# gopro/cineform-sdk

Measured on AMD Instinct MI355X. Metric: 1080p YUY2 encode+decode fps, higher is better.
Workload: dtype int16

## Files before the change

cineform-sdk_amd/csrc/cfhd_batch.cpp:

```cpp
#include "../../include/cfhd_amd.h"
#include "cfhd_core.h"
#include "cfhd_bitstream.h"
#include "cfhd_device.h"
#include "cfhd_metadata.h"
#include "cfhd_params.h"
#include <string.h>
#include <stdlib.h>
#include <vector>
#include <thread>
#include <atomic>
#include <chrono>
#include <memory>

using namespace cfhd;

struct cfhd_amd_chunk { EncodeBatch enc; DecodeBatch dec; int first = 0, n = 0; };

struct cfhd_amd_batch {
	FramePlan plan;
	int n = 0, nthreads = 1, quality = 4, pixel_kind = PIX_YUY2;
	int color_format = 2, color_space = 2; bool progressive = true;
	bool decode = true;
	std::vector<std::unique_ptr<cfhd_amd_chunk>> chunks;
	cfhd_amd_chunk &chunk_of(int i, int *local) { for (auto &c : chunks) if (i < c->first + c->n) { *local = i - c->first; return *c; } *local = 0; return *chunks[0]; }
// ... 36 lines not shown
	static const int forced = [] { const char *e = getenv("CFHD_AMD_QUEUE"); return e && strcmp(e, "ordered") == 0 ? 2 : (e && strcmp(e, "free") == 0 ? 0 : -1); }();
	const int turns = forced >= 0 ? forced : (b->decode ? 0 : 1);
	const bool ordered = turns >= 1, ordered_decode = turns >= 2;
	if (ordered && stage_order_wait(c->enc.device(), 0, c->enc.stream())) return -2;
	if (b->host_in && c->enc.upload_frames(b->host_in, b->host_in_stride, b->host_in_pitch)) return -2;
	if (c->enc.launch_forward(false)) return -2;
	for (int l = 0; l < c->n; l++) {
		SampleHeaderInfo h = { base_number + (uint32_t)(c->first + l) + 1, b->color_format, b->color_space, b->quality, b->progressive, b->frame_meta[c->first + l].data(), b->frame_meta[c->first + l].size(), nullptr, 0 };
		if (c->enc.entropy().set_frame_header(l, h)) return -6;
	}
	if (c->enc.entropy().launch()) return -2;
	if (ordered && stage_order_done(c->enc.device(), 0, c->enc.stream())) return -2;
	if (b->decode) {
		if (ordered_decode && stage_order_wait(c->enc.device(), 1, c->dec.stream())) return -5;
		c->dec.entropy().set_producer_events(c->enc.entropy().headers_event(), c->enc.entropy().samples_event());
		if (c->dec.entropy().set_samples_device(c->enc.entropy().device_sample(0), c->enc.entropy().sample_cap(), c->enc.entropy().device_sizes())) return -4;
		if (c->dec.launch_entropy() || c->dec.launch_inverse(seed + (uint32_t)c->first)) return -5;
		if (ordered_decode && stage_order_done(c->enc.device(), 1, c->dec.stream())) return -5;
		if (b->host_out && c->dec.download_frames(b->host_out, b->host_out_stride, b->host_out_pitch)) return -5;
	}
	if (c->enc.entropy().download_queue()) return -2;
	b->t_launched = now();
	return 0;
}
long long batch_finish(cfhd_amd_batch *b)
{
	cfhd_amd_chunk *c = b->chunks[0].get();
	if (c->enc.entropy().download_finish() || c->enc.wait()) return -2;
	bool overflow = false, peaks = false;
	for (int l = 0; l < c->n; l++) {
		size_t n = c->enc.entropy().sample_bytes(l); b->sample_size[c->first + l] = n;
// ... 112 lines not shown
		const int rc = batch_launch(b);
		if (rc) return rc;
		return batch_finish(b);
	} else if (b->gpu_entropy && b->device_handoff) {
		prepare_meta();
		std::atomic<int> err(0);
		std::vector<double> t_sub(b->chunks.size(), 0.0), t_enc(b->chunks.size(), 0.0);
		parallel_for((int)b->chunks.size(), (int)b->chunks.size(), [&](int k) {
			cfhd_amd_chunk *c = b->chunks[k].get();
			auto fail = [&](int code) { int z = 0; err.compare_exchange_strong(z, code); };
			if (c->enc.launch_forward(false)) return fail(-2);
			for (int l = 0; l < c->n; l++) if (c->enc.entropy().set_frame_header(l, header(c->first + l))) return fail(-6);
			if (c->enc.entropy().launch()) return fail(-2);
			if (b->decode) {
				c->dec.entropy().set_producer_events(c->enc.entropy().headers_event(), c->enc.entropy().samples_event());
				if (c->dec.entropy().set_samples_device(c->enc.entropy().device_sample(0), c->enc.entropy().sample_cap(), c->enc.entropy().device_sizes())) return fail(-4);
				if (c->dec.launch_entropy() || c->dec.launch_inverse(seed + (uint32_t)c->first)) return fail(-5);
			}
			t_sub[k] = now();
			if (c->enc.entropy().download() || c->enc.wait()) return fail(-2);
			for (int l = 0; l < c->n; l++) {
				size_t n = c->enc.entropy().sample_bytes(l); b->sample_size[c->first + l] = n; if (!n) { fail(-3); continue; }
				if (c->enc.entropy().needs_peak_table(l)) fail(-8);
			}
			t_enc[k] = now();
			if (b->decode) { if (c->dec.wait()) return fail(-5); if (c->dec.entropy().check()) return fail(-7); }
		});
		if (err.load()) return err.load();
		t1 = t0; t2 = t0;
		for (size_t k = 0; k < b->chunks.size(); k++) { if (t_sub[k] > t1) t1 = t_sub[k]; if (t_enc[k] > t2) t2 = t_enc[k]; }
		if (t2 < t1) t2 = t1;
// ... 188 lines not shown
```

cineform-sdk_amd/csrc/cfhd_entropy_gpu.h:

```cpp
#pragma once
#include "cfhd_core.h"
#include "cfhd_bitstream.h"
#include "cfhd_gop.h"
#include <vector>

namespace cfhd {

int device_stream_create(void **stream);
void device_stream_destroy(void *stream);
void device_stream_release(void *stream);
void device_streams_lean(bool on);
bool device_streams_are_lean();
struct StreamScope { StreamScope(); explicit StreamScope(void *preset ); ~StreamScope(); void *stream() const; };


class GpuEntropyEncoder {
public:
	GpuEntropyEncoder();
	~GpuEntropyEncoder();
	int prepare(const FramePlan &plan, int nframes, int16_t *d_coeffs, size_t coeff_stride_elems, size_t sample_cap, void *stream);
	int set_frame_header(int i, const SampleHeaderInfo &hdr);
	void set_plan(const FramePlan &plan) { plan_ = plan; }
	int prepare_group(const GopPlan &plan, int ngroups, int16_t *d_coeffs, size_t coeff_stride_elems, size_t sample_cap, void *stream);
	void set_group_plan(const GopPlan &plan) { gplan_ = plan; }
	int launch();
	int download();
	int download_queue();
	int download_finish();
	int fetch_sizes();
	const uint32_t *device_sizes() const { return d_sizes_; }
	const uint8_t *host_sample(int i) const { return h_samples_ + h_offsets_[i]; }
	uint8_t *device_sample(int i) { return d_samples_ + (size_t)i * cap_; }
	uint32_t sample_bytes(int i) const { return h_sizes_[i]; }
	void set_active(int k) { active_ = k; }
	void set_speculative_download(bool on) { speculative_download_ = on; if (!on) expect_bytes_ = 0; }
	bool needs_peak_table(int i) const { return peak_flags_in_use() && (h_sizes_[n_ + i] & 2u) != 0; }
	bool has_peak_table(int i) const { return peak_flags_in_use() && (h_sizes_[n_ + i] & 1u) != 0; }
	bool peak_flags_in_use() const { return group_ ? gplan_.interlaced : plan_.interlaced; }
	size_t sample_cap() const { return cap_; }
	int total_segments() const { return total_segs_; }
	float kernel_ms(int k);
	void set_level1_event(void *ev) { ev_level1_ = ev; }
	void *block_slots() const { return d_blocks_; }
	unsigned long long *block_masks(int frame) const { return d_masks_ ? d_masks_ + (size_t)frame * masks_per_frame_ : nullptr; }
	void set_block_lists(bool on) { use_blocks_ = on && d_blocks_; }
	bool block_lists() const { return use_blocks_; }
	void *headers_event() const { return ev_[3]; }
	void *samples_event() const { return ev_[4]; }
private:
	struct Host; Host *host_;
	void release();
	int prepare_units(int n, int16_t *d_coeffs, size_t coeff_stride_elems, size_t sample_cap, void *stream);
	void build_template(const SampleHeaderInfo &hdr, SampleTemplate *t) const;
	bool group_ = false; GopPlan gplan_;
	FramePlan plan_; int n_ = 0, active_ = 0, device_ = 0 ; size_t cap_ = 0; void *stream_ = nullptr;
	int active_frames() const { return active_ > 0 && active_ < n_ ? active_ : n_; }
	int nbands_ = 0, total_segs_ = 0; size_t tok_per_frame_ = 0;
	std::vector<SampleTemplate> tmpl_;
	uint8_t *d_samples_ = nullptr, *h_samples_ = nullptr;
	uint32_t *d_sizes_ = nullptr, *h_sizes_ = nullptr;
	uint8_t *d_packed_ = nullptr; uint32_t *d_offsets_ = nullptr, *h_offsets_ = nullptr;
	size_t expect_bytes_ = 0, copied_ahead_ = 0; int expect_frames_ = 0; bool speculative_download_ = false;
	void *d_tables_ = nullptr, *d_bands_ = nullptr, *d_segband_ = nullptr, *d_segs_ = nullptr, *d_bandstate_ = nullptr, *d_frames_ = nullptr, *d_tokens_ = nullptr;
	uint8_t *d_tmpl_ = nullptr, *h_tmpl_ = nullptr;
	bool dirty_ = true;
	void *ev_[5] = {nullptr, nullptr, nullptr, nullptr, nullptr}; bool timed_ = false;
	bool split_ = false, serial_split_ = false; void *ev_level1_ = nullptr, *stream2_ = nullptr, *ev2_[3] = {nullptr, nullptr, nullptr};
	int16_t *d_coeffs_ = nullptr; size_t coeff_stride_ = 0;
	void *d_blocks_ = nullptr; unsigned long long *d_masks_ = nullptr; size_t masks_per_frame_ = 0; bool use_blocks_ = false;
};


class GpuEntropyDecoder {
public:
	GpuEntropyDecoder();
	~GpuEntropyDecoder();
	void set_interlaced(bool on) { interlaced_ = on; }
	void set_active(int k) { active_ = k; }
	void set_skip_level1(bool skip) { skip_level1_ = skip; }
	int prepare(const FramePlan &plan, int nframes, int16_t *d_coeffs, size_t coeff_stride_elems, size_t sample_cap, int out_pixel_kind, void *stream);
	int set_sample_host(int i, const uint8_t *sample, size_t size);
	int set_sample_device(int i, const uint8_t *d_sample, const uint8_t *host_copy, size_t size);
	int set_samples_device(const uint8_t *d_samples, size_t stride_bytes, const uint32_t *d_sizes);
	void set_producer_events(void *headers, void *payloads) { ev_headers_ = headers; ev_payloads_ = payloads; }
	int launch();
	int check();
	float kernel_ms(int k);
	bool chunk_indexed() const { return dx_; }
	void *levels23_event() const { return l23_split_ ? ev_l23_ : nullptr; }
	void set_block_lists(bool on) { use_blocks_ = on && d_masks_; }
	bool level1_as_block_lists() const { return blocks_written_; }
	void dense_pyramid_uploaded() { blocks_written_ = false; }
	const unsigned long long *block_masks(int frame) const { return d_masks_ ? d_masks_ + (size_t)frame * masks_per_frame_ : nullptr; }
	int stats(uint32_t out[16]);
private:
	struct Host; Host *host_;
	void release();
	FramePlan plan_; int n_ = 0, out_kind_ = 0; size_t cap_ = 0, coeff_stride_ = 0; void *stream_ = nullptr;
	int16_t *d_coeffs_ = nullptr;
	uint8_t *d_samples_ = nullptr, *h_samples_ = nullptr;
	void *d_tables_ = nullptr, *d_bandjobs_ = nullptr, *d_lowjobs_ = nullptr, *d_plan_ = nullptr;
	void *ev_headers_ = nullptr, *ev_payloads_ = nullptr;
	bool skip_level1_ = false, interlaced_ = false; void *d_diffjobs_ = nullptr;
	int active_ = 0;
	int active_frames() const { return active_ > 0 && active_ < n_ ? active_ : n_; }
	const uint8_t *ext_samples_ = nullptr; size_t ext_stride_ = 0; const uint32_t *ext_sizes_ = nullptr;
	int *d_errors_ = nullptr, *h_errors_ = nullptr;
	bool lane_kernel_ = false;
	bool dx_ = true;
	void *d_tile_start_ = nullptr, *d_stats_ = nullptr, *d_repair_ = nullptr, *d_alts_ = nullptr, *d_reindex_ = nullptr, *d_alt_entries_ = nullptr; uint32_t alt_slots_ = 0;
	void *d_idx_tables_ = nullptr, *d_entries_ = nullptr, *d_recs_ = nullptr, *d_chunk_base_ = nullptr, *d_chunk_job_ = nullptr, *d_sums_ = nullptr, *d_counters_ = nullptr;
	uint32_t max_chunks_ = 0, *h_counters_ = nullptr; void *h_chunk_job_ = nullptr;
	int grid_index_ = 0, grid_tiles_ = 0;
	int device_ = 0;
	int launch_dx(bool device_jobs, int njobs, uint32_t host_chunks, int lowpass_jobs);
	void *ev_l23_ = nullptr, *ev_low_ = nullptr; bool l23_split_ = false;
	void *ev_[8] = {nullptr, nullptr, nullptr, nullptr, nullptr, nullptr, nullptr, nullptr}; bool timed_ = false;
	bool parse_end_ = false;
	unsigned long long *d_masks_ = nullptr; size_t masks_per_frame_ = 0; bool use_blocks_ = false, blocks_written_ = false;
};

// ... 19 lines not shown
```

cineform-sdk_amd/csrc/cfhd_entropy_gpu.hip:

```cpp
#include "cfhd_entropy_gpu.h"
#include "cfhd_entropy_jobs.h"
#include <hip/hip_runtime.h>
#include <string.h>
#include <stdio.h>
#include <stdlib.h>
#include <algorithm>

namespace cfhd {

int device_init();
int device_current();
namespace { int g_fail(hipError_t e, const char *what) { fprintf(stderr, "[cfhd_amd] %s: %s\n", what, hipGetErrorString(e)); return (int)e ? (int)e : -1; } }
#define HIPCHK(expr) do { hipError_t _e = (expr); if (_e != hipSuccess) return g_fail(_e, #expr); } while (0)

struct GpuEntropyEncoder::Host { EntHostJobs jobs; std::vector<EntHoleGeom> geom; dev::EntFrameJob *frames = nullptr;  };

GpuEntropyEncoder::GpuEntropyEncoder() : host_(new Host) {}
GpuEntropyEncoder::~GpuEntropyEncoder() { release(); delete host_; }

void GpuEntropyEncoder::release()
{
	(void)hipSetDevice(device_);
	void *dev[] = { d_samples_, d_sizes_, d_tables_, d_bands_, d_segband_, d_segs_, d_bandstate_, d_frames_, d_tmpl_, d_packed_, d_offsets_, d_tokens_, d_blocks_, d_masks_ };
	for (void *p : dev) if (p) (void)hipFree(p);
	if (h_samples_) (void)hipHostFree(h_samples_);
	if (h_sizes_) (void)hipHostFree(h_sizes_);
	if (h_offsets_) (void)hipHostFree(h_offsets_);
	d_packed_ = nullptr; d_offsets_ = h_offsets_ = nullptr;
	if (h_tmpl_) (void)hipHostFree(h_tmpl_);
	if (host_->frames) { (void)hipHostFree(host_->frames); host_->frames = nullptr; }
	for (void *&e : ev_) if (e) { (void)hipEventDestroy((hipEvent_t)e); e = nullptr; }
	for (void *&e : ev2_) if (e) { (void)hipEventDestroy((hipEvent_t)e); e = nullptr; }
	if (stream2_) { device_stream_destroy(stream2_); stream2_ = nullptr; }
	timed_ = false;
	d_samples_ = h_samples_ = nullptr; d_sizes_ = h_sizes_ = nullptr; d_tables_ = d_bands_ = d_segband_ = d_segs_ = d_bandstate_ = d_frames_ = d_tokens_ = nullptr;
	d_tmpl_ = h_tmpl_ = nullptr; n_ = 0;
	d_blocks_ = nullptr; d_masks_ = nullptr; masks_per_frame_ = 0; use_blocks_ = false;
}

int GpuEntropyEncoder::prepare(const FramePlan &plan, int nframes, int16_t *d_coeffs, size_t stride, size_t sample_cap, void *stream)
{
	group_ = false; plan_ = plan;
	return prepare_units(nframes, d_coeffs, stride, sample_cap, stream);
}

int GpuEntropyEncoder::prepare_group(const GopPlan &plan, int ngroups, int16_t *d_coeffs, size_t stride, size_t sample_cap, void *stream)
{
	group_ = true; gplan_ = plan; plan_ = FramePlan(); plan_.interlaced = false;
	return prepare_units(ngroups, d_coeffs, stride, sample_cap, stream);
}
// ... 31 lines not shown
	HIPCHK(hipMalloc(&d_bands_, jobs.bands.size() * sizeof(dev::EntBandJob)));
	HIPCHK(hipMemcpy(d_bands_, jobs.bands.data(), jobs.bands.size() * sizeof(dev::EntBandJob), hipMemcpyHostToDevice));
	HIPCHK(hipMalloc(&d_segband_, jobs.segjobs.size() * sizeof(dev::EntSegJob)));
	HIPCHK(hipMemcpy(d_segband_, jobs.segjobs.data(), jobs.segjobs.size() * sizeof(dev::EntSegJob), hipMemcpyHostToDevice));
	HIPCHK(hipMalloc(&d_segs_, jobs.segjobs.size() * sizeof(dev::EntSegState)));
	HIPCHK(hipMalloc(&d_tokens_, jobs.tok_per_frame * (size_t)n_ * sizeof(uint32_t)));
	HIPCHK(hipMalloc(&d_bandstate_, jobs.bands.size() * sizeof(dev::EntBandState)));
	static_assert((int)kBlockChunkCols == (int)dev::FWD_CHUNK_COLS_ENT, "one chunk geometry");
	if (lists) {
		int mask_base[kMaxChannels][kNumBands];
		masks_per_frame_ = (size_t)block_list_layout(plan, mask_base);
		HIPCHK(hipMalloc(&d_blocks_, stride * 2 * (size_t)n_));
		HIPCHK(hipMalloc((void **)&d_masks_, masks_per_frame_ * 8 * (size_t)n_ + 64));
		HIPCHK(hipMemset(d_masks_, 0, masks_per_frame_ * 8 * (size_t)n_ + 64));
	}
	HIPCHK(hipMalloc((void **)&d_samples_, cap_ * n_));
	HIPCHK(hipHostMalloc((void **)&h_samples_, cap_ * n_, hipHostMallocPortable));
	HIPCHK(hipMalloc((void **)&d_sizes_, sizeof(uint32_t) * 2 * n_));
	HIPCHK(hipHostMalloc((void **)&h_sizes_, sizeof(uint32_t) * 2 * n_, hipHostMallocPortable));
	memset(h_sizes_, 0, sizeof(uint32_t) * 2 * n_);
	HIPCHK(hipMalloc((void **)&d_packed_, cap_ * n_));
	HIPCHK(hipMalloc((void **)&d_offsets_, sizeof(uint32_t) * (n_ + 1)));
	HIPCHK(hipHostMalloc((void **)&h_offsets_, sizeof(uint32_t) * (n_ + 1), hipHostMallocPortable));
	memset(h_offsets_, 0, sizeof(uint32_t) * (n_ + 1));
	HIPCHK(hipMalloc((void **)&d_tmpl_, (size_t)kEntTmplStride * n_));
	HIPCHK(hipHostMalloc((void **)&h_tmpl_, (size_t)kEntTmplStride * n_, hipHostMallocPortable));
	memset(h_tmpl_, 0, (size_t)kEntTmplStride * n_);
	HIPCHK(hipMalloc(&d_frames_, n_ * sizeof(dev::EntFrameJob)));
	HIPCHK(hipHostMalloc((void **)&host_->frames, n_ * sizeof(dev::EntFrameJob), hipHostMallocPortable));
	for (int f = 0; f < n_; f++) { SampleHeaderInfo h = hdr0; h.frame_number = (uint32_t)f + 1; if ((rc = set_frame_header(f, h))) return rc; }
	for (void *&e : ev_) HIPCHK(hipEventCreate((hipEvent_t *)&e));
	for (void *&e : ev2_) HIPCHK(hipEventCreate((hipEvent_t *)&e));
	if (n_ >= 8 || !device_streams_are_lean()) HIPCHK((hipError_t)device_stream_create(&stream2_));
	return 0;
}

int GpuEntropyEncoder::set_frame_header(int f, const SampleHeaderInfo &hdr)
{
	if (f < 0 || f >= n_) return -1;
	SampleTemplate &t = tmpl_[f];
	build_template(hdr, &t);
	if (!ent_fill_frame_block(host_->geom, t, f, host_->jobs, d_coeffs_ + (size_t)f * coeff_stride_, h_tmpl_ + (size_t)kEntTmplStride * f)) return -4;
	host_->frames[f] = ent_frame_job(t, d_tmpl_ + (size_t)kEntTmplStride * f, d_samples_ + cap_ * f, (uint32_t)cap_, d_sizes_ + f, d_sizes_ + n_ + f);
	dirty_ = true;
	return 0;
}

int GpuEntropyEncoder::launch()
{
	(void)hipSetDevice(device_);
	hipStream_t st = (hipStream_t)stream_;
	if (dirty_) {
		HIPCHK(hipMemcpyAsync(d_tmpl_, h_tmpl_, (size_t)kEntTmplStride * n_, hipMemcpyHostToDevice, st));
		HIPCHK(hipMemcpyAsync(d_frames_, host_->frames, n_ * sizeof(dev::EntFrameJob), hipMemcpyHostToDevice, st));
		dirty_ = false;
	}
	const dev::EntTables *T = (const dev::EntTables *)d_tables_;
	const dev::EntBatchGeom geom = { total_segs_ / n_, nbands_, coeff_stride_, tok_per_frame_ };
// ... 31 lines not shown
		HIPCHK(hipStreamWaitEvent(s2, (hipEvent_t)ev_level1_, 0));
		if (peak_flags_in_use()) HIPCHK(hipMemsetAsync(d_sizes_ + n_, 0, sizeof(uint32_t) * n_, s2));
		HIPCHK(hipEventRecord((hipEvent_t)ev2_[0], s2));
		for (const auto &r : host_->jobs.ranges_l1) count_range(s2, r.first, r.second, true);
		HIPCHK(hipEventRecord((hipEvent_t)ev2_[1], s2));
		for (const auto &r : host_->jobs.ranges_rest) count_range(st, r.first, r.second);
		HIPCHK(hipEventRecord((hipEvent_t)ev2_[2], st));
		HIPCHK(hipStreamWaitEvent(st, (hipEvent_t)ev2_[1], 0));
	} else if (use_blocks_) {
		for (const auto &r : host_->jobs.ranges_l1) count_range(st, r.first, r.second, true);
		for (const auto &r : host_->jobs.ranges_rest) count_range(st, r.first, r.second);
	} else count_range(st, 0, total_segs_ / n_);
	HIPCHK(hipEventRecord((hipEvent_t)ev_[1], st));
	dev::k_ent_scan<<<nbands_ * act, dev::ENT_THREADS, 0, st>>>((const dev::EntBandJob *)d_bands_, (dev::EntSegState *)d_segs_, (dev::EntBandState *)d_bandstate_, T);
	HIPCHK(hipEventRecord((hipEvent_t)ev_[2], st));
	const unsigned layout_parts = act >= 256 ? 8u : (unsigned)((2048 + act - 1) / act > 256 ? 256 : (2048 + act - 1) / act);
	dev::k_ent_layout<<<dim3((unsigned)act, layout_parts), dev::ENT_THREADS, 0, st>>>((const dev::EntFrameJob *)d_frames_, (const dev::EntBandJob *)d_bands_, (dev::EntSegState *)d_segs_,
	                                                  (dev::EntBandState *)d_bandstate_, T);
	HIPCHK(hipEventRecord((hipEvent_t)ev_[3], st));
	{
		dev::EntPeakHoles which; which.n = 0;
		for (size_t h = 0; h < tmpl_[0].holes.size() && which.n < 7; h++) if (tmpl_[0].holes[h].kind == 2) which.hole[which.n++] = (int)h;
		if (which.n) dev::k_ent_peaks<<<dim3(act >= 64 ? 4u : 32u, (unsigned)which.n, (unsigned)act), dev::ENT_THREADS, 0, st>>>((const dev::EntFrameJob *)d_frames_, which, (const dev::EntBandJob *)d_bands_,
		                                                  (const dev::EntSegJob *)d_segband_, geom, (const dev::EntSegState *)d_segs_, (const dev::EntBandState *)d_bandstate_);
	}
#ifdef CFHD_AMD_PROBES
	const int emit_probe = []{ const char *e = getenv("CFHD_AMD_EMIT_PROBE"); return e ? atoi(e) : 0; }();
#else
	const int emit_probe = 0;
#endif
// ... 23 lines not shown
{
	(void)hipSetDevice(device_);
	hipStream_t st = (hipStream_t)stream_;
	HIPCHK(hipMemcpyAsync(h_sizes_, d_sizes_, sizeof(uint32_t) * 2 * n_, hipMemcpyDeviceToHost, st));
	HIPCHK(hipStreamSynchronize(st));
	return 0;
}

int GpuEntropyEncoder::download() { const int rc = download_queue(); return rc ? rc : download_finish(); }

int GpuEntropyEncoder::download_queue()
{
	(void)hipSetDevice(device_);
	hipStream_t st = (hipStream_t)stream_;
	const bool direct = false;
	(void)hipGetLastError();
	const int act = active_frames();
	dev::k_ent_pack_offsets<<<1, dev::ENT_THREADS, 0, st>>>(d_sizes_, act, d_offsets_);
	dev::k_ent_pack<<<dim3(direct ? 2 : 8, (unsigned)act), dev::ENT_THREADS, 0, st>>>(d_samples_, cap_, d_sizes_, d_offsets_, direct ? h_samples_ : d_packed_);
	HIPCHK(hipGetLastError());
	HIPCHK(hipMemcpyAsync(h_sizes_, d_sizes_, sizeof(uint32_t) * 2 * n_, hipMemcpyDeviceToHost, st));
	HIPCHK(hipMemcpyAsync(h_offsets_, d_offsets_, sizeof(uint32_t) * (act + 1), hipMemcpyDeviceToHost, st));
	copied_ahead_ = 0;
	if (!direct && expect_bytes_ && expect_frames_ == act) {
		copied_ahead_ = expect_bytes_ < cap_ * (size_t)act ? expect_bytes_ : cap_ * (size_t)act;
		HIPCHK(hipMemcpyAsync(h_samples_, d_packed_, copied_ahead_, hipMemcpyDeviceToHost, st));
	}
	return 0;
}

int GpuEntropyEncoder::download_finish()
{
	(void)hipSetDevice(device_);
	hipStream_t st = (hipStream_t)stream_;
	const bool direct = false;
// ... 103 lines not shown
		HIPCHK(hipMalloc(&d_plan_, sizeof(dp)));
		HIPCHK(hipMemcpy(d_plan_, &dp, sizeof(dp), hipMemcpyHostToDevice));
	}
	if (dx_ && plan.encoded_format == ENC_YUV422 && plan.num_channels == 3) {
		int mask_base[kMaxChannels][kNumBands];
		masks_per_frame_ = (size_t)dec_block_list_layout(plan, mask_base);
		HIPCHK(hipMalloc((void **)&d_masks_, masks_per_frame_ * 8 * (size_t)n_));
	}
	host_->bands.assign(n_, {}); host_->lows.assign(n_, {}); host_->diffs.assign(n_, {}); host_->host_bytes.assign(n_, 0);
	for (void *&e : ev_) HIPCHK(hipEventCreate((hipEvent_t *)&e));
	HIPCHK(hipEventCreate((hipEvent_t *)&ev_l23_));
	HIPCHK(hipEventCreate((hipEvent_t *)&ev_low_));
	return 0;
}

int GpuEntropyDecoder::set_samples_device(const uint8_t *d_samples, size_t stride_bytes, const uint32_t *d_sizes)
{
	if (!d_samples || !d_sizes || (stride_bytes & 255) || ((uintptr_t)d_samples & 255)) return -1;
	ext_samples_ = d_samples; ext_stride_ = stride_bytes; ext_sizes_ = d_sizes;
	return 0;
}

int GpuEntropyDecoder::set_sample_host(int i, const uint8_t *sample, size_t size)
{
	if (i < 0 || i >= n_ || size > cap_) return -1;
	memcpy(h_samples_ + cap_ * i, sample, size);
	int rc = set_sample_device(i, d_samples_ + cap_ * i, sample, size);
	if (rc == 0) host_->host_bytes[i] = (size + 3) & ~(size_t)3;
	return rc;
}

int GpuEntropyDecoder::set_sample_device(int i, const uint8_t *d_sample, const uint8_t *host_copy, size_t size)
{
	if (i < 0 || i >= n_) return -1;
// ... 21 lines not shown
int GpuEntropyDecoder::launch()
{
	(void)hipSetDevice(device_);
	hipStream_t st = (hipStream_t)stream_;
	l23_split_ = false; blocks_written_ = false;
	if (ext_samples_) {
		const int nch = plan_.num_channels, nb = n_ * nch * 9;
		HIPCHK(hipMemsetAsync(d_errors_, 0, sizeof(int), st));
		(void)hipGetLastError();
		static const bool parse_early = [] { const char *e = getenv("CFHD_AMD_PARSE_EARLY"); return !(e && atoi(e) == 0); }();
		if (!parse_early && ev_payloads_) ev_headers_ = ev_payloads_;
		if (ev_headers_) HIPCHK(hipStreamWaitEvent(st, (hipEvent_t)ev_headers_, 0));
		HIPCHK(hipEventRecord((hipEvent_t)ev_[0], st));
		dev::k_dec_parse<<<n_, dev::DEC_PARSE_THREADS, 0, st>>>(ext_samples_, ext_stride_, ext_sizes_, n_,
			(const dev::DecPlan *)d_plan_, d_coeffs_, coeff_stride_, (dev::DecBandJob *)d_bandjobs_, (dev::DecLowpassJob *)d_lowjobs_, d_errors_,
			interlaced_ && dx_ ? (dev::DecDiffJob *)d_diffjobs_ : nullptr);
		parse_end_ = ev_payloads_ != nullptr;
		if (parse_end_) { HIPCHK(hipEventRecord((hipEvent_t)ev_[4], st)); HIPCHK(hipStreamWaitEvent(st, (hipEvent_t)ev_payloads_, 0)); }
		ev_headers_ = ev_payloads_ = nullptr;
		HIPCHK(hipEventRecord((hipEvent_t)ev_[1], st));
		l23_split_ = false;
		if (dx_) { const int rc_dx = launch_dx(true, nb, 0u, n_ * nch); if (rc_dx) return rc_dx; }
		else if (n_ <= kLowLatencyFrames) dev::k_dec_bands_par_ll<<<nb, dev::DECP_LL_THREADS, 0, st>>>((const dev::DecBandJob *)d_bandjobs_, (const dev::DecTables *)d_tables_, d_errors_);
		else dev::k_dec_bands_par<<<nb, dev::DECP_THREADS, 0, st>>>((const dev::DecBandJob *)d_bandjobs_, (const dev::DecTables *)d_tables_, d_errors_);
		HIPCHK(hipEventRecord((hipEvent_t)ev_[2], st));
		if (!l23_split_) dev::k_dec_lowpass<<<dim3(8, (unsigned)(n_ * nch)), 256, 0, st>>>((const dev::DecLowpassJob *)d_lowjobs_);
		HIPCHK(hipGetLastError());
		HIPCHK(hipEventRecord((hipEvent_t)ev_[3], st));
		timed_ = true;
		HIPCHK(hipMemcpyAsync(h_errors_, d_errors_, sizeof(int), hipMemcpyDeviceToHost, st));
		return 0;
// ... 269 lines not shown
```

cineform-sdk_amd/csrc/cfhd_entropy_jobs.h:

```cpp
#pragma once
#include "cfhd_core.h"
#include "cfhd_bitstream.h"
#include "cfhd_gop.h"
#include "cfhd_entropy_kernels.h"
#include "cfhd_dec_kernels.h"
#include <vector>
#include <algorithm>
#include <string.h>

namespace cfhd {

enum { kEntTmplBytes = 6144, kEntWordHolesBytes = 1536, kEntHolesBytes = dev::ENT_MAX_HOLES * (int)sizeof(dev::EntHole), kEntMaxPatches = 96,
       kEntPatchBytes = kEntMaxPatches * (int)sizeof(dev::EntPatch), kEntTmplStride = kEntTmplBytes + kEntWordHolesBytes + kEntHolesBytes + kEntPatchBytes };

inline void ent_build_tables(dev::EntTables *h, int codebook = 1)
{
	const EntropyTables *t = entropy_tables(codebook);
	memcpy(h->value_code, t->value_code, sizeof(h->value_code));
	memcpy(h->run_bits, t->run_bits, sizeof(h->run_bits));
	for (int c = 0; c < 3072; c++) { h->run_count[c] = t->run_count[c]; h->run_size[c] = t->run_size[c]; }
	h->run_total[0] = 0;
	for (int c = 1; c < 3072; c++) h->run_total[c] = (uint16_t)(t->run_size[c] + h->run_total[c - t->run_count[c]]);
	h->band_end_bits = t->band_end_bits; h->band_end_size = t->band_end_size;
	for (int c = 0; c < 3072; c++) { h->run_pack[c].x = t->run_bits[c]; h->run_pack[c].y = (uint32_t)t->run_size[c] | ((uint32_t)t->run_count[c] << 8); }
// ... 271 lines not shown
		d.lp_width = bd.width; d.lp_height = bd.height; d.lp_pitch = bd.pitch;
	}
	dev::EntPatch *ep = (dev::EntPatch *)(block + kEntTmplBytes + kEntWordHolesBytes + kEntHolesBytes);
	for (size_t i = 0; i < t.patches.size(); i++) {
		const SampleTemplate::Patch &p = t.patches[i];
		ep[i].kind = p.kind; ep[i].at_tmpl = p.at_tmpl; ep[i].at_holes = p.at_holes; ep[i].start_tmpl = p.start_tmpl; ep[i].start_holes = p.start_holes;
		ep[i].end_tmpl = p.end_tmpl; ep[i].end_holes = p.end_holes; ep[i].tag = p.tag;
	}
	return true;
}
inline bool ent_fill_frame_block(const FramePlan &plan, const SampleTemplate &t, int f, const EntHostJobs &jobs, const int16_t *coeffs_f, uint8_t *block)
{
	return ent_fill_frame_block(ent_hole_geometry(plan, t), t, f, jobs, coeffs_f, block);
}

inline dev::EntFrameJob ent_frame_job(const SampleTemplate &t, uint8_t *block_addr, uint8_t *out, uint32_t out_cap, uint32_t *size_out, uint32_t *peak_flag)
{
	dev::EntFrameJob fj;
	fj.out = out; fj.out_cap = out_cap;
	fj.tmpl = block_addr; fj.tmpl_bytes = (int)t.bytes.size();
	fj.word_holes = block_addr + kEntTmplBytes;
	fj.holes = (const dev::EntHole *)(block_addr + kEntTmplBytes + kEntWordHolesBytes); fj.nholes = (int)t.holes.size();
	fj.patches = (const dev::EntPatch *)(block_addr + kEntTmplBytes + kEntWordHolesBytes + kEntHolesBytes); fj.npatches = (int)t.patches.size();
	fj.sample_bytes = size_out; fj.peak_flag = peak_flag;
	return fj;
}


inline bool dec_build_jobs(const ParsedSample &ps, const FramePlan &plan, const uint8_t *sample_addr, int16_t *coeff_base, int out_pixel_kind,
                           std::vector<dev::DecBandJob> *bands, std::vector<dev::DecLowpassJob> *lowpass, bool skip_level1 = false)
{
	for (int c = 0; c < plan.num_channels; c++) {
		const ParsedBand &lp = ps.lowpass[c];
		const BandDesc &ll = plan.ch[c].band[2][0];
// ... 113 lines not shown
```

cineform-sdk_amd/csrc/cfhd_entropy_kernels.h:

```cpp
#pragma once
#include <stdint.h>
#include <cfhd_gfx950.h>

#ifdef CFHD_AMD_PROBES
#define CFHD_PROBE(p) (p)
#else
#define CFHD_PROBE(p) 0
#endif

namespace cfhd {
namespace dev {

#ifndef CFHD_ENT_FILL
#define CFHD_ENT_FILL 16384
#endif
#ifndef CFHD_ENT_PER_THREAD
#define CFHD_ENT_PER_THREAD 16
#endif
#ifndef CFHD_ENT_TOK_CAP
#define CFHD_ENT_TOK_CAP 256
#endif
enum { FWD_CHUNK_COLS_ENT = 496 };
enum { ENT_THREADS = 256, ENT_LANES = 64, ENT_WAVES = ENT_THREADS / ENT_LANES, ENT_PER_THREAD = CFHD_ENT_PER_THREAD, ENT_SEG = ENT_LANES * ENT_PER_THREAD,
       ENT_LDS_WORDS = 1024, ENT_TOK_CAP = CFHD_ENT_TOK_CAP, ENT_MAX_HOLES = 60 ,
// ... 53 lines not shown

struct EntBandState { uint32_t seg_bits, tail_run, payload_bytes, base_byte; uint8_t *out;
                      uint32_t npeaks, pad; uint8_t *peak_out;  };

struct EntHole { int tmpl_offset, kind, fixed_bytes, band_job; const int16_t *lowpass; int lp_width, lp_height, lp_pitch; };
struct EntPatch { int kind, at_tmpl, at_holes, start_tmpl, start_holes, end_tmpl, end_holes, tag; };

struct EntFrameJob {
	uint8_t *out; uint32_t out_cap;
	const uint8_t *tmpl; int tmpl_bytes;
	const uint8_t *word_holes;
	const EntHole *holes; int nholes;
	const EntPatch *patches; int npatches;
	uint32_t *sample_bytes;
	uint32_t *peak_flag;
};

__device__ __forceinline__ uint32_t bswap32(uint32_t v) { return (v >> 24) | ((v >> 8) & 0xff00u) | ((v << 8) & 0xff0000u) | (v << 24); }

__device__ __forceinline__ int block_excl_sum(int v, int *buf, int *total)
{
	const int lane = wave_lane(), wave = (int)(threadIdx.x >> 6);
	const int incl = (int)wave_incl_scan((uint32_t)v);
	if (lane == ENT_LANES - 1) buf[wave] = incl;
	__syncthreads();
	int base = 0, tot = 0;
#pragma unroll
	for (int w = 0; w < ENT_WAVES; w++) { const int x = buf[w]; if (w < wave) base += x; tot += x; }
	if (total) *total = tot;
	__syncthreads();
// ... 359 lines not shown
		b.base_byte = 0; b.out = nullptr;
		b.npeaks = carry_peaks; b.pad = 0; b.peak_out = nullptr;
	}
}

__device__ __forceinline__ void put_code_plain(uint32_t *words, uint64_t pos, uint32_t code, int size)
{
	if (!size) return;
	const uint64_t v = (uint64_t)code << (64 - size - (int)(pos & 31));
	uint32_t *w = words + (pos >> 5);
	w[0] |= bswap32((uint32_t)(v >> 32));
	const uint32_t lo = (uint32_t)v;
	if (lo) w[1] |= bswap32(lo);
}

__global__ void __launch_bounds__(ENT_THREADS) k_ent_layout(const EntFrameJob *frames, const EntBandJob *bands, EntSegState *segs,
                                                             EntBandState *band_state, const EntTables *tables)
{
	const EntFrameJob &f = frames[blockIdx.x];
	const int part = blockIdx.y, nparts = gridDim.y;
	__shared__ uint32_t s_cum[ENT_MAX_HOLES + 1];
	__shared__ uint32_t s_piece[ENT_MAX_HOLES + 1];
	__shared__ int s_ok;
	const int tid = threadIdx.x;
	if (tid < 64) {
		uint32_t bytes = 0;
		if (tid < f.nholes) {
			const EntHole &hole = f.holes[tid];
			if (hole.kind == 0) bytes = (uint32_t)hole.fixed_bytes;
			else if (hole.kind == 1) bytes = band_state[hole.band_job].payload_bytes;
			else {
				const uint32_t np = band_state[hole.band_job].npeaks;
				bytes = (np && np <= (uint32_t)ENT_PEAK_TABLE_MAX) ? 4u + 4u * ((np + 1u) >> 1) : 0u;
			}
		}
		const uint32_t pieces = tid < f.nholes ? (bytes / ENT_FILL ? bytes / ENT_FILL : 1u) : 0u;
		const uint32_t cum = wave_incl_scan(bytes), pc = wave_incl_scan(pieces);
		if (tid <= f.nholes && tid <= ENT_MAX_HOLES) { s_cum[tid] = cum - bytes; s_piece[tid] = pc - pieces; }
		const uint32_t total = (uint32_t)f.tmpl_bytes + wave_get(cum, 63);
		if (tid == 0) { s_ok = total <= f.out_cap; if (part == 0) *f.sample_bytes = total <= f.out_cap ? total : 0u; }
	}
	__syncthreads();
	if (!s_ok) return;
	uint32_t *out = (uint32_t *)f.out;
	const uint32_t *tw = (const uint32_t *)f.tmpl;
	if (part == 0) for (int i = tid; i < f.tmpl_bytes / 4; i += ENT_THREADS) out[i + (s_cum[f.word_holes[i]] >> 2)] = tw[i];
	__syncthreads();
	for (int i = tid; part == 0 && i < f.npatches; i += ENT_THREADS) {
		const EntPatch &p = f.patches[i];
		const uint32_t at = (uint32_t)p.at_tmpl + s_cum[p.at_holes], end = (uint32_t)p.end_tmpl + s_cum[p.end_holes];
		if (p.kind == 0) {
			uint32_t size = (end - at) >> 2; size = size ? size - 1 : 0;
			int tag = p.tag;
			if (tag & 0x2000) { tag |= (int)((size >> 16) & 0xff); size &= 0xffff; } else size &= 0xffff;
			tag = -tag;
			out[at >> 2] = bswap32(((uint32_t)(uint16_t)tag << 16) | size);
		} else if (p.kind == 2) {
			if (s_cum[p.start_holes + 1] != s_cum[p.start_holes]) {
				const uint32_t offset = end - at;
// ... 20 lines not shown
				uint32_t w = 0;
#pragma unroll
				for (int q = 0; q < 2; q++) {
					const int e = 2 * (int)i + q;
					uint32_t v = 0;
					if (e < count) { const int r = e / hole.lp_width, c = e - r * hole.lp_width; v = (uint16_t)hole.lowpass[(size_t)r * hole.lp_pitch + c]; }
					w = (w << 16) | v;
				}
				out[(base >> 2) + i] = bswap32(w);
			}
			continue;
		}
		if (hole.kind == 2) {
			const uint32_t np = band_state[hole.band_job].npeaks;
			for (uint32_t i = w0 + tid; i < w1; i += ENT_THREADS) out[(base >> 2) + i] = i == 0 ? bswap32(((uint32_t)(uint16_t)(-0x4001) << 16) | ((np + 1u) >> 1)) : 0u;
			if (k == 0 && tid == 0) band_state[hole.band_job].peak_out = bytes ? f.out + base + 4 : nullptr;
			continue;
		}
		const EntBandState bs = band_state[hole.band_job];
		const uint32_t tail_word = (uint32_t)(bs.seg_bits >> 5) < bytes / 4 ? (uint32_t)(bs.seg_bits >> 5) : bytes / 4;
		for (uint32_t i = w0 + tid; i < (w1 < tail_word ? w1 : tail_word); i += ENT_THREADS) out[(base >> 2) + i] = 0;
		if (k != last) continue;
		const EntTables *T = tables + bands[hole.band_job].table;
		const uint32_t maxc = T->run_count[3071], maxs = T->run_size[3071], maxb = T->run_bits[3071];
		const uint32_t copies = bs.tail_run >= 3071u ? (bs.tail_run - 3071u) / maxc + 1u : 0u;
		const uint64_t p0 = bs.seg_bits, p1 = p0 + (uint64_t)copies * maxs;
		uint32_t *words = out + (base >> 2);
		for (uint32_t i = tail_word + tid; i < bytes / 4; i += ENT_THREADS) {
			uint32_t w = 0;
			const uint64_t lo = (uint64_t)i * 32u, hi = lo + 32u;
			if (copies && hi > p0 && lo < p1) {
				uint64_t j = lo > p0 ? (lo - p0) / maxs : 0u;
				for (; j < copies && p0 + j * maxs < hi; j++) {
					const int64_t sh = (int64_t)(hi - (p0 + j * maxs)) - (int64_t)maxs;
					w |= sh >= 0 ? (sh < 32 ? maxb << sh : 0u) : maxb >> (-sh);
				}
			}
			words[i] = bswap32(w);
		}
		__syncthreads();
		for (int i = tid; i < bands[hole.band_job].nseg; i += ENT_THREADS) segs[bands[hole.band_job].seg_base + i].out = f.out + base;
		if (tid == 0) {
			EntBandState &b = band_state[hole.band_job];
			b.base_byte = base; b.out = f.out + base;
			uint64_t pos = p1;
			uint32_t run = bs.tail_run - copies * maxc;
			while (run > 0) {
				const uint32_t idx = run < 3072 ? run : 3071;
				put_code_plain(words, pos, T->run_bits[idx], T->run_size[idx]);
				pos += T->run_size[idx];
				run -= T->run_count[idx];
			}
			put_code_plain(words, pos, T->band_end_bits, T->band_end_size);
		}
	}
}

__device__ __forceinline__ void ent_put_string(uint32_t *s_words, uint32_t *out, bool use_lds, uint32_t first_word, uint64_t pos, uint64_t str)
{
// ... 184 lines not shown
__global__ void __launch_bounds__(ENT_THREADS) k_ent_pack_offsets(const uint32_t *sizes, int n, uint32_t *offsets)
{
	__shared__ int s_scan[ENT_THREADS];
	uint32_t carry = 0;
	for (int c0 = 0; c0 < n; c0 += ENT_THREADS) {
		const int i = c0 + (int)threadIdx.x;
		const uint32_t sz = i < n ? (sizes[i] + 63u) & ~63u : 0u;
		int total;
		const uint32_t off = carry + (uint32_t)block_excl_sum((int)sz, s_scan, &total);
		if (i < n) offsets[i] = off;
		carry += (uint32_t)total;
	}
	if (threadIdx.x == 0) offsets[n] = carry;
}

__global__ void __launch_bounds__(ENT_THREADS) k_ent_pack(const uint8_t *samples, size_t stride, const uint32_t *sizes, const uint32_t *offsets, uint8_t *packed)
{
	const int f = blockIdx.y;
	const uint4 *src = (const uint4 *)(samples + stride * (size_t)f);
	uint4 *dst = (uint4 *)(packed + offsets[f]);
	const uint32_t n16 = (sizes[f] + 15u) >> 4;
	for (uint32_t i = blockIdx.x * ENT_THREADS + threadIdx.x; i < n16; i += gridDim.x * ENT_THREADS) dst[i] = src[i];
}

enum { DEC_K1 = 12, DEC_THREADS = 64 };

struct DecMulti {
	uint16_t pre_bits;
	int16_t v1;
	uint16_t mid_post;
	int16_t v2;
};

struct DecTables {
	DecMulti multi[1 << DEC_K1];
	uint32_t lut1[1 << DEC_K1];
	uint32_t lut2_size;
	uint32_t lut2[1];
};
// ... 198 lines not shown
};
enum { DEC_PARSE_THREADS = 64, DEC_ERR_PARSE = 0x100 };

struct DecTagReader {
	const uint8_t *d; uint64_t base; uint32_t w; int lane;
	__device__ __forceinline__ uint32_t word(uint64_t pos)
	{
		const uint64_t b = pos & ~(uint64_t)255;
		if (b != base) { w = *(const uint32_t *)(d + b + 4 * (size_t)lane); base = b; }
		return bswap32(wave_read(w, (int)((pos >> 2) & 63u)));
	}
};

__global__ void __launch_bounds__(DEC_PARSE_THREADS) k_dec_parse(const uint8_t *samples, size_t sample_stride, const uint32_t *sizes, int nframes, const DecPlan *P,
                                                                 int16_t *coeffs, size_t coeff_stride, DecBandJob *bandjobs, DecLowpassJob *lowjobs, int *errors,
                                                                 DecDiffJob *diffjobs )
{
	const int f = blockIdx.x;
	const int lane = wave_lane();
	const bool writer = lane == 0;
	const uint8_t *d = samples + sample_stride * (size_t)f;
	int16_t *cbase = coeffs + coeff_stride * (size_t)f;
	const uint64_t size = sizes[f];
	const int nch = P->num_channels;
	if (writer) for (int c = 0; c < nch; c++) {
		lowjobs[f * nch + c] = DecLowpassJob{ d, cbase + P->low[c].offset, 0, 0, P->low[c].pitch, 0 };
		for (int lv = 0; lv < 3; lv++)
			for (int b = 1; b < 4; b++) {
				const DecPlanBand pb = P->high[c][lv][b];
				bandjobs[(size_t)P->slot[c][lv][b] * nframes + f] = DecBandJob{ d, 0u, cbase + pb.offset, pb.height * pb.pitch, 1 };
			}
	}
	DecTagReader rd; rd.d = d; rd.base = ~(uint64_t)0; rd.w = 0; rd.lane = lane;
	uint64_t pos = 0, pending_at = 0, peak_base = 0;
	uint32_t pending = 0, seen_low = 0, peak_offset = 0;
	int peak_level = 0;
// ... 97 lines not shown
```

Before: 66320.

## Write encoded samples directly into packed buffer, drop separate pack kernel

Sample sizes and dense offsets are now computed before the layout kernel, so the encoder writes each frame's bitstream straight into the packed output buffer instead of a per-frame strided buffer. This removes the k_ent_pack copy kernel and the strided sample allocation, and the decoder reads samples through the offset table. It adds a small sizes kernel and moves the offset scan earlier in the stream. The size computation is now done twice (once in the sizes kernel, once in layout).

```diff
diff --git a/cineform-sdk_amd/csrc/cfhd_batch.cpp b/cineform-sdk_amd/csrc/cfhd_batch.cpp
--- a/cineform-sdk_amd/csrc/cfhd_batch.cpp
+++ b/cineform-sdk_amd/csrc/cfhd_batch.cpp
@@ -74,7 +74,7 @@
 	if (b->decode) {
 		if (ordered_decode && stage_order_wait(c->enc.device(), 1, c->dec.stream())) return -5;
 		c->dec.entropy().set_producer_events(c->enc.entropy().headers_event(), c->enc.entropy().samples_event());
-		if (c->dec.entropy().set_samples_device(c->enc.entropy().device_sample(0), c->enc.entropy().sample_cap(), c->enc.entropy().device_sizes())) return -4;
+		if (c->dec.entropy().set_samples_device(c->enc.entropy().device_samples(), 0, c->enc.entropy().device_sizes(), c->enc.entropy().device_offsets())) return -4;
 		if (c->dec.launch_entropy() || c->dec.launch_inverse(seed + (uint32_t)c->first)) return -5;
 		if (ordered_decode && stage_order_done(c->enc.device(), 1, c->dec.stream())) return -5;
 		if (b->host_out && c->dec.download_frames(b->host_out, b->host_out_stride, b->host_out_pitch)) return -5;
@@ -217,7 +217,7 @@
 			if (c->enc.entropy().launch()) return fail(-2);
 			if (b->decode) {
 				c->dec.entropy().set_producer_events(c->enc.entropy().headers_event(), c->enc.entropy().samples_event());
-				if (c->dec.entropy().set_samples_device(c->enc.entropy().device_sample(0), c->enc.entropy().sample_cap(), c->enc.entropy().device_sizes())) return fail(-4);
+				if (c->dec.entropy().set_samples_device(c->enc.entropy().device_samples(), 0, c->enc.entropy().device_sizes(), c->enc.entropy().device_offsets())) return fail(-4);
 				if (c->dec.launch_entropy() || c->dec.launch_inverse(seed + (uint32_t)c->first)) return fail(-5);
 			}
 			t_sub[k] = now();
diff --git a/cineform-sdk_amd/csrc/cfhd_entropy_gpu.h b/cineform-sdk_amd/csrc/cfhd_entropy_gpu.h
--- a/cineform-sdk_amd/csrc/cfhd_entropy_gpu.h
+++ b/cineform-sdk_amd/csrc/cfhd_entropy_gpu.h
@@ -30,7 +30,8 @@
 	int fetch_sizes();
 	const uint32_t *device_sizes() const { return d_sizes_; }
 	const uint8_t *host_sample(int i) const { return h_samples_ + h_offsets_[i]; }
-	uint8_t *device_sample(int i) { return d_samples_ + (size_t)i * cap_; }
+	const uint8_t *device_samples() const { return d_packed_; }
+	const uint32_t *device_offsets() const { return d_offsets_; }
 	uint32_t sample_bytes(int i) const { return h_sizes_[i]; }
 	void set_active(int k) { active_ = k; }
 	void set_speculative_download(bool on) { speculative_download_ = on; if (!on) expect_bytes_ = 0; }
@@ -57,7 +58,7 @@
 	int active_frames() const { return active_ > 0 && active_ < n_ ? active_ : n_; }
 	int nbands_ = 0, total_segs_ = 0; size_t tok_per_frame_ = 0;
 	std::vector<SampleTemplate> tmpl_;
-	uint8_t *d_samples_ = nullptr, *h_samples_ = nullptr;
+	uint8_t *h_samples_ = nullptr;
 	uint32_t *d_sizes_ = nullptr, *h_sizes_ = nullptr;
 	uint8_t *d_packed_ = nullptr; uint32_t *d_offsets_ = nullptr, *h_offsets_ = nullptr;
 	size_t expect_bytes_ = 0, copied_ahead_ = 0; int expect_frames_ = 0; bool speculative_download_ = false;
@@ -81,7 +82,7 @@
 	int prepare(const FramePlan &plan, int nframes, int16_t *d_coeffs, size_t coeff_stride_elems, size_t sample_cap, int out_pixel_kind, void *stream);
 	int set_sample_host(int i, const uint8_t *sample, size_t size);
 	int set_sample_device(int i, const uint8_t *d_sample, const uint8_t *host_copy, size_t size);
-	int set_samples_device(const uint8_t *d_samples, size_t stride_bytes, const uint32_t *d_sizes);
+	int set_samples_device(const uint8_t *d_samples, size_t stride_bytes, const uint32_t *d_sizes, const uint32_t *d_offsets = nullptr);
 	void set_producer_events(void *headers, void *payloads) { ev_headers_ = headers; ev_payloads_ = payloads; }
 	int launch();
 	int check();
@@ -104,7 +105,7 @@
 	bool skip_level1_ = false, interlaced_ = false; void *d_diffjobs_ = nullptr;
 	int active_ = 0;
 	int active_frames() const { return active_ > 0 && active_ < n_ ? active_ : n_; }
-	const uint8_t *ext_samples_ = nullptr; size_t ext_stride_ = 0; const uint32_t *ext_sizes_ = nullptr;
+	const uint8_t *ext_samples_ = nullptr; size_t ext_stride_ = 0; const uint32_t *ext_sizes_ = nullptr, *ext_offsets_ = nullptr;
 	int *d_errors_ = nullptr, *h_errors_ = nullptr;
 	bool lane_kernel_ = false;
 	bool dx_ = true;
diff --git a/cineform-sdk_amd/csrc/cfhd_entropy_gpu.hip b/cineform-sdk_amd/csrc/cfhd_entropy_gpu.hip
--- a/cineform-sdk_amd/csrc/cfhd_entropy_gpu.hip
+++ b/cineform-sdk_amd/csrc/cfhd_entropy_gpu.hip
@@ -21,7 +21,7 @@
 void GpuEntropyEncoder::release()
 {
 	(void)hipSetDevice(device_);
-	void *dev[] = { d_samples_, d_sizes_, d_tables_, d_bands_, d_segband_, d_segs_, d_bandstate_, d_frames_, d_tmpl_, d_packed_, d_offsets_, d_tokens_, d_blocks_, d_masks_ };
+	void *dev[] = { d_sizes_, d_tables_, d_bands_, d_segband_, d_segs_, d_bandstate_, d_frames_, d_tmpl_, d_packed_, d_offsets_, d_tokens_, d_blocks_, d_masks_ };
 	for (void *p : dev) if (p) (void)hipFree(p);
 	if (h_samples_) (void)hipHostFree(h_samples_);
 	if (h_sizes_) (void)hipHostFree(h_sizes_);
@@ -33,7 +33,7 @@
 	for (void *&e : ev2_) if (e) { (void)hipEventDestroy((hipEvent_t)e); e = nullptr; }
 	if (stream2_) { device_stream_destroy(stream2_); stream2_ = nullptr; }
 	timed_ = false;
-	d_samples_ = h_samples_ = nullptr; d_sizes_ = h_sizes_ = nullptr; d_tables_ = d_bands_ = d_segband_ = d_segs_ = d_bandstate_ = d_frames_ = d_tokens_ = nullptr;
+	h_samples_ = nullptr; d_sizes_ = h_sizes_ = nullptr; d_tables_ = d_bands_ = d_segband_ = d_segs_ = d_bandstate_ = d_frames_ = d_tokens_ = nullptr;
 	d_tmpl_ = h_tmpl_ = nullptr; n_ = 0;
 	d_blocks_ = nullptr; d_masks_ = nullptr; masks_per_frame_ = 0; use_blocks_ = false;
 }
@@ -95,12 +95,11 @@
 		HIPCHK(hipMalloc((void **)&d_masks_, masks_per_frame_ * 8 * (size_t)n_ + 64));
 		HIPCHK(hipMemset(d_masks_, 0, masks_per_frame_ * 8 * (size_t)n_ + 64));
 	}
-	HIPCHK(hipMalloc((void **)&d_samples_, cap_ * n_));
 	HIPCHK(hipHostMalloc((void **)&h_samples_, cap_ * n_, hipHostMallocPortable));
 	HIPCHK(hipMalloc((void **)&d_sizes_, sizeof(uint32_t) * 2 * n_));
 	HIPCHK(hipHostMalloc((void **)&h_sizes_, sizeof(uint32_t) * 2 * n_, hipHostMallocPortable));
 	memset(h_sizes_, 0, sizeof(uint32_t) * 2 * n_);
-	HIPCHK(hipMalloc((void **)&d_packed_, cap_ * n_));
+	HIPCHK(hipMalloc((void **)&d_packed_, cap_ * n_ + 256));
 	HIPCHK(hipMalloc((void **)&d_offsets_, sizeof(uint32_t) * (n_ + 1)));
 	HIPCHK(hipHostMalloc((void **)&h_offsets_, sizeof(uint32_t) * (n_ + 1), hipHostMallocPortable));
 	memset(h_offsets_, 0, sizeof(uint32_t) * (n_ + 1));
@@ -122,7 +121,7 @@
 	SampleTemplate &t = tmpl_[f];
 	build_template(hdr, &t);
 	if (!ent_fill_frame_block(host_->geom, t, f, host_->jobs, d_coeffs_ + (size_t)f * coeff_stride_, h_tmpl_ + (size_t)kEntTmplStride * f)) return -4;
-	host_->frames[f] = ent_frame_job(t, d_tmpl_ + (size_t)kEntTmplStride * f, d_samples_ + cap_ * f, (uint32_t)cap_, d_sizes_ + f, d_sizes_ + n_ + f);
+	host_->frames[f] = ent_frame_job(t, d_tmpl_ + (size_t)kEntTmplStride * f, d_packed_, (uint32_t)cap_, d_sizes_ + f, d_sizes_ + n_ + f, d_offsets_ + f);
 	dirty_ = true;
 	return 0;
 }
@@ -184,6 +183,8 @@
 	HIPCHK(hipEventRecord((hipEvent_t)ev_[1], st));
 	dev::k_ent_scan<<<nbands_ * act, dev::ENT_THREADS, 0, st>>>((const dev::EntBandJob *)d_bands_, (dev::EntSegState *)d_segs_, (dev::EntBandState *)d_bandstate_, T);
 	HIPCHK(hipEventRecord((hipEvent_t)ev_[2], st));
+	dev::k_ent_sizes<<<(act + dev::ENT_WAVES - 1) / dev::ENT_WAVES, dev::ENT_THREADS, 0, st>>>((const dev::EntFrameJob *)d_frames_, act, (const dev::EntBandState *)d_bandstate_);
+	dev::k_ent_pack_offsets<<<1, dev::ENT_THREADS, 0, st>>>(d_sizes_, act, d_offsets_);
 	const unsigned layout_parts = act >= 256 ? 8u : (unsigned)((2048 + act - 1) / act > 256 ? 256 : (2048 + act - 1) / act);
 	dev::k_ent_layout<<<dim3((unsigned)act, layout_parts), dev::ENT_THREADS, 0, st>>>((const dev::EntFrameJob *)d_frames_, (const dev::EntBandJob *)d_bands_, (dev::EntSegState *)d_segs_,
 	                                                  (dev::EntBandState *)d_bandstate_, T);
@@ -237,11 +238,7 @@
 	(void)hipSetDevice(device_);
 	hipStream_t st = (hipStream_t)stream_;
 	const bool direct = false;
-	(void)hipGetLastError();
 	const int act = active_frames();
-	dev::k_ent_pack_offsets<<<1, dev::ENT_THREADS, 0, st>>>(d_sizes_, act, d_offsets_);
-	dev::k_ent_pack<<<dim3(direct ? 2 : 8, (unsigned)act), dev::ENT_THREADS, 0, st>>>(d_samples_, cap_, d_sizes_, d_offsets_, direct ? h_samples_ : d_packed_);
-	HIPCHK(hipGetLastError());
 	HIPCHK(hipMemcpyAsync(h_sizes_, d_sizes_, sizeof(uint32_t) * 2 * n_, hipMemcpyDeviceToHost, st));
 	HIPCHK(hipMemcpyAsync(h_offsets_, d_offsets_, sizeof(uint32_t) * (act + 1), hipMemcpyDeviceToHost, st));
 	copied_ahead_ = 0;
@@ -375,10 +372,10 @@
 	return 0;
 }
 
-int GpuEntropyDecoder::set_samples_device(const uint8_t *d_samples, size_t stride_bytes, const uint32_t *d_sizes)
-{
-	if (!d_samples || !d_sizes || (stride_bytes & 255) || ((uintptr_t)d_samples & 255)) return -1;
-	ext_samples_ = d_samples; ext_stride_ = stride_bytes; ext_sizes_ = d_sizes;
+int GpuEntropyDecoder::set_samples_device(const uint8_t *d_samples, size_t stride_bytes, const uint32_t *d_sizes, const uint32_t *d_offsets)
+{
+	if (!d_samples || !d_sizes || ((uintptr_t)d_samples & 255) || (!d_offsets && (stride_bytes & 255))) return -1;
+	ext_samples_ = d_samples; ext_stride_ = stride_bytes; ext_sizes_ = d_sizes; ext_offsets_ = d_offsets;
 	return 0;
 }
 
@@ -430,7 +427,7 @@
 		HIPCHK(hipEventRecord((hipEvent_t)ev_[0], st));
 		dev::k_dec_parse<<<n_, dev::DEC_PARSE_THREADS, 0, st>>>(ext_samples_, ext_stride_, ext_sizes_, n_,
 			(const dev::DecPlan *)d_plan_, d_coeffs_, coeff_stride_, (dev::DecBandJob *)d_bandjobs_, (dev::DecLowpassJob *)d_lowjobs_, d_errors_,
-			interlaced_ && dx_ ? (dev::DecDiffJob *)d_diffjobs_ : nullptr);
+			interlaced_ && dx_ ? (dev::DecDiffJob *)d_diffjobs_ : nullptr, ext_offsets_);
 		parse_end_ = ev_payloads_ != nullptr;
 		if (parse_end_) { HIPCHK(hipEventRecord((hipEvent_t)ev_[4], st)); HIPCHK(hipStreamWaitEvent(st, (hipEvent_t)ev_payloads_, 0)); }
 		ev_headers_ = ev_payloads_ = nullptr;
diff --git a/cineform-sdk_amd/csrc/cfhd_entropy_jobs.h b/cineform-sdk_amd/csrc/cfhd_entropy_jobs.h
--- a/cineform-sdk_amd/csrc/cfhd_entropy_jobs.h
+++ b/cineform-sdk_amd/csrc/cfhd_entropy_jobs.h
@@ -309,10 +309,10 @@
 	return ent_fill_frame_block(ent_hole_geometry(plan, t), t, f, jobs, coeffs_f, block);
 }
 
-inline dev::EntFrameJob ent_frame_job(const SampleTemplate &t, uint8_t *block_addr, uint8_t *out, uint32_t out_cap, uint32_t *size_out, uint32_t *peak_flag)
+inline dev::EntFrameJob ent_frame_job(const SampleTemplate &t, uint8_t *block_addr, uint8_t *out, uint32_t out_cap, uint32_t *size_out, uint32_t *peak_flag, const uint32_t *dense_off = nullptr)
 {
 	dev::EntFrameJob fj;
-	fj.out = out; fj.out_cap = out_cap;
+	fj.out = out; fj.out_cap = out_cap; fj.dense_off = dense_off;
 	fj.tmpl = block_addr; fj.tmpl_bytes = (int)t.bytes.size();
 	fj.word_holes = block_addr + kEntTmplBytes;
 	fj.holes = (const dev::EntHole *)(block_addr + kEntTmplBytes + kEntWordHolesBytes); fj.nholes = (int)t.holes.size();
diff --git a/cineform-sdk_amd/csrc/cfhd_entropy_kernels.h b/cineform-sdk_amd/csrc/cfhd_entropy_kernels.h
--- a/cineform-sdk_amd/csrc/cfhd_entropy_kernels.h
+++ b/cineform-sdk_amd/csrc/cfhd_entropy_kernels.h
@@ -91,6 +91,7 @@
 	const EntPatch *patches; int npatches;
 	uint32_t *sample_bytes;
 	uint32_t *peak_flag;
+	const uint32_t *dense_off;
 };
 
 __device__ __forceinline__ uint32_t bswap32(uint32_t v) { return (v >> 24) | ((v >> 8) & 0xff00u) | ((v << 8) & 0xff0000u) | (v << 24); }
@@ -480,6 +481,33 @@
 	if (lo) w[1] |= bswap32(lo);
 }
 
+__device__ __forceinline__ uint32_t ent_sample_size(const EntFrameJob &f, const EntBandState *band_state, int lane, uint32_t *hole_bytes, uint32_t *cum_incl)
+{
+	uint32_t bytes = 0;
+	if (lane < f.nholes) {
+		const EntHole &hole = f.holes[lane];
+		if (hole.kind == 0) bytes = (uint32_t)hole.fixed_bytes;
+		else if (hole.kind == 1) bytes = band_state[hole.band_job].payload_bytes;
+		else {
+			const uint32_t np = band_state[hole.band_job].npeaks;
+			bytes = (np && np <= (uint32_t)ENT_PEAK_TABLE_MAX) ? 4u + 4u * ((np + 1u) >> 1) : 0u;
+		}
+	}
+	const uint32_t cum = wave_incl_scan(bytes);
+	*hole_bytes = bytes; *cum_incl = cum;
+	return (uint32_t)f.tmpl_bytes + wave_get(cum, 63);
+}
+
+__global__ void __launch_bounds__(ENT_THREADS) k_ent_sizes(const EntFrameJob *frames, int nframes, const EntBandState *band_state)
+{
+	const int fr = wave_uniform((int)(blockIdx.x * ENT_WAVES + (threadIdx.x >> 6)));
+	if (fr >= nframes) return;
+	const EntFrameJob &f = frames[fr];
+	uint32_t bytes, cum;
+	const uint32_t total = ent_sample_size(f, band_state, wave_lane(), &bytes, &cum);
+	if (wave_lane() == 0) *f.sample_bytes = total <= f.out_cap ? total : 0u;
+}
+
 __global__ void __launch_bounds__(ENT_THREADS) k_ent_layout(const EntFrameJob *frames, const EntBandJob *bands, EntSegState *segs,
                                                              EntBandState *band_state, const EntTables *tables)
 {
@@ -490,25 +518,17 @@
 	__shared__ int s_ok;
 	const int tid = threadIdx.x;
 	if (tid < 64) {
-		uint32_t bytes = 0;
-		if (tid < f.nholes) {
-			const EntHole &hole = f.holes[tid];
-			if (hole.kind == 0) bytes = (uint32_t)hole.fixed_bytes;
-			else if (hole.kind == 1) bytes = band_state[hole.band_job].payload_bytes;
-			else {
-				const uint32_t np = band_state[hole.band_job].npeaks;
-				bytes = (np && np <= (uint32_t)ENT_PEAK_TABLE_MAX) ? 4u + 4u * ((np + 1u) >> 1) : 0u;
-			}
-		}
+		uint32_t bytes, cum;
+		const uint32_t total = ent_sample_size(f, band_state, tid, &bytes, &cum);
 		const uint32_t pieces = tid < f.nholes ? (bytes / ENT_FILL ? bytes / ENT_FILL : 1u) : 0u;
-		const uint32_t cum = wave_incl_scan(bytes), pc = wave_incl_scan(pieces);
+		const uint32_t pc = wave_incl_scan(pieces);
 		if (tid <= f.nholes && tid <= ENT_MAX_HOLES) { s_cum[tid] = cum - bytes; s_piece[tid] = pc - pieces; }
-		const uint32_t total = (uint32_t)f.tmpl_bytes + wave_get(cum, 63);
 		if (tid == 0) { s_ok = total <= f.out_cap; if (part == 0) *f.sample_bytes = total <= f.out_cap ? total : 0u; }
 	}
 	__syncthreads();
 	if (!s_ok) return;
-	uint32_t *out = (uint32_t *)f.out;
+	uint8_t *const fout = f.out + (f.dense_off ? *f.dense_off : 0u);
+	uint32_t *out = (uint32_t *)fout;
 	const uint32_t *tw = (const uint32_t *)f.tmpl;
 	if (part == 0) for (int i = tid; i < f.tmpl_bytes / 4; i += ENT_THREADS) out[i + (s_cum[f.word_holes[i]] >> 2)] = tw[i];
 	__syncthreads();
@@ -559,7 +579,7 @@
 		if (hole.kind == 2) {
 			const uint32_t np = band_state[hole.band_job].npeaks;
 			for (uint32_t i = w0 + tid; i < w1; i += ENT_THREADS) out[(base >> 2) + i] = i == 0 ? bswap32(((uint32_t)(uint16_t)(-0x4001) << 16) | ((np + 1u) >> 1)) : 0u;
-			if (k == 0 && tid == 0) band_state[hole.band_job].peak_out = bytes ? f.out + base + 4 : nullptr;
+			if (k == 0 && tid == 0) band_state[hole.band_job].peak_out = bytes ? fout + base + 4 : nullptr;
 			continue;
 		}
 		const EntBandState bs = band_state[hole.band_job];
@@ -584,10 +604,10 @@
 			words[i] = bswap32(w);
 		}
 		__syncthreads();
-		for (int i = tid; i < bands[hole.band_job].nseg; i += ENT_THREADS) segs[bands[hole.band_job].seg_base + i].out = f.out + base;
+		for (int i = tid; i < bands[hole.band_job].nseg; i += ENT_THREADS) segs[bands[hole.band_job].seg_base + i].out = fout + base;
 		if (tid == 0) {
 			EntBandState &b = band_state[hole.band_job];
-			b.base_byte = base; b.out = f.out + base;
+			b.base_byte = base; b.out = fout + base;
 			uint64_t pos = p1;
 			uint32_t run = bs.tail_run - copies * maxc;
 			while (run > 0) {
@@ -802,15 +822,6 @@
 	if (threadIdx.x == 0) offsets[n] = carry;
 }
 
-__global__ void __launch_bounds__(ENT_THREADS) k_ent_pack(const uint8_t *samples, size_t stride, const uint32_t *sizes, const uint32_t *offsets, uint8_t *packed)
-{
-	const int f = blockIdx.y;
-	const uint4 *src = (const uint4 *)(samples + stride * (size_t)f);
-	uint4 *dst = (uint4 *)(packed + offsets[f]);
-	const uint32_t n16 = (sizes[f] + 15u) >> 4;
-	for (uint32_t i = blockIdx.x * ENT_THREADS + threadIdx.x; i < n16; i += gridDim.x * ENT_THREADS) dst[i] = src[i];
-}
-
 enum { DEC_K1 = 12, DEC_THREADS = 64 };
 
 struct DecMulti {
@@ -1039,12 +1050,13 @@
 
 __global__ void __launch_bounds__(DEC_PARSE_THREADS) k_dec_parse(const uint8_t *samples, size_t sample_stride, const uint32_t *sizes, int nframes, const DecPlan *P,
                                                                  int16_t *coeffs, size_t coeff_stride, DecBandJob *bandjobs, DecLowpassJob *lowjobs, int *errors,
-                                                                 DecDiffJob *diffjobs )
+                                                                 DecDiffJob *diffjobs ,
+                                                                 const uint32_t *offsets = nullptr )
 {
 	const int f = blockIdx.x;
 	const int lane = wave_lane();
 	const bool writer = lane == 0;
-	const uint8_t *d = samples + sample_stride * (size_t)f;
+	const uint8_t *d = offsets ? samples + offsets[f] : samples + sample_stride * (size_t)f;
 	int16_t *cbase = coeffs + coeff_stride * (size_t)f;
 	const uint64_t size = sizes[f];
 	const int nch = P->num_channels;
```

New measurement: 67000 (median of 6 runs). 1.01x the previous value.
